# zhejz/TrafficBotsV1.5

Hardware: AMD Instinct MI355X
Metric: sim-agent-steps/sec (closed-loop rollout) (higher is better)
Workload: dtype f32 (split-bf16 MFMA products); 1 GPU; 64-agent/1024-polyline/128-light synthetic scene, 5-step teacher-forced prime + 1047-step closed-loop rollout; scenes_per_gpu=1, graph=True, steps_per_graph_replay=40, pre_roll_rollouts=32, one_queue_paired_launches=True, attn_mfma=False

## Files before the change

trafficbotsv1.5_amd/csrc/front.hip:

```cpp
#include <string.h>

#include "knn_core.h"
#include "tile_core.h"
#include "window_core.h"

using namespace tbx_tile;

namespace {

typedef Planes<16, 4> RPL;
constexpr int XLD = 132;
constexpr size_t WIN_BYTES = tbx_window::LDS_BYTES;
constexpr size_t POOL_OFF = WIN_BYTES;
constexpr size_t ROWP_OFF = POOL_OFF + 2 * D * sizeof(float);
constexpr size_t WIN_TOTAL = ROWP_OFF + 4 * 512;
constexpr size_t RIDER_TOTAL = 16 * XLD * sizeof(float) + 4 * RPL::PLANE;
constexpr size_t LDS_BYTES = WIN_TOTAL > RIDER_TOTAL ? WIN_TOTAL : RIDER_TOTAL;

struct FrontArgs {
  tbx_window_tile_t win;
  tbx_layer_tile_t lt;
  tbx_knn::KnnMulti knn;
  int n_win_blocks, n_rider_blocks, n_knn_blocks;
};

__device__ __forceinline__ void proj_rows(const tbx_layer_tile_t& t, const int block, const float* pooled, char* rowp) {
  const int tid = (int)threadIdx.x, lane = tid & 63;
  const int wave = __builtin_amdgcn_readfirstlane(tid >> 6);
  const int g4 = lane >> 4;
  const bool col0 = (lane & 15) == 0;
  const int c_out = 16 * wave + 4 * g4;
  constexpr int LO = 256;
  char* Ph = rowp;
  char* Pq = rowp + 1024;
  W wb[2];
  load_unit(wb[0], t.proj_image, wave, lane);
  load_unit(wb[1], t.proj_image, 8 + wave, lane);
  if (wave < 2) row1::ln_planes(pooled + wave * D, Ph + wave * 512, lane, t.proj_norm_eps, t.proj_norm_weight, t.proj_norm_bias);
  __syncthreads();
  const int64_t row0 = (int64_t)block * 2;
  const int nv = (t.n_rows - row0) < 2 ? (int)(t.n_rows - row0) : 2;
#pragma unroll
  for (int r = 0; r < 2; ++r) {
    const f32x4 q = row1::gemv4(wb[0], Ph + r * 512, LO, 0, g4) + wb[0].bias;
    if (col0) {
      row1::put4(Pq + r * 512, LO, c_out, q);
      if (r < nv) gst4(t.proj_out + (row0 + r) * (int64_t)t.ld_proj + c_out, q);
    }
  }
  load_unit(wb[0], t.proj_image, 16 + wave, lane);
#pragma unroll
  for (int kv = 0; kv < 2; ++kv) {
    const W& w = wb[1 - kv];
#pragma unroll
    for (int r = 0; r < 2; ++r) {
      const f32x4 y = row1::gemv4(w, Ph + r * 512, LO, 0, g4) + w.bias;
      if (col0 && r < nv) {
        gst4(t.proj_out + (row0 + r) * (int64_t)t.ld_proj + (1 + kv) * D + c_out, y);
        if (t.kv16_out != nullptr) {
          const bf16x4 h16 = __builtin_convertvector(y, bf16x4);
          *(TBX_GLOBAL u32x2*)((uint16_t*)t.kv16_out + (row0 + r) * (2 * D) + kv * D + c_out) = __builtin_bit_cast(u32x2, h16);
        }
      }
    }
    if (kv == 0) load_unit(wb[1], t.qfold_image, wave, lane);
  }
  __syncthreads();
  {
    const W& w = wb[1];
    const int h = wave >> 1;
#pragma unroll
    for (int st = 0; st < 4; ++st)
#pragma unroll
      for (int r = 0; r < 2; ++r) {
        Acc acc;
        acc.zero();
        row1::step(acc, w.hi[st], w.lo[st], Pq + r * 512, LO, h, g4);
        if (col0 && r < nv) gst4(t.proj_out + (row0 + r) * (int64_t)t.ld_proj + 3 * D + h * D + ((wave & 1) * 4 + st) * 16 + 4 * g4, acc.sum());
      }
  }
}

template <int DM, bool ADD>
__device__ __forceinline__ void front_body(const FrontArgs& a, int b, char* lds_c) {
  if (b < a.n_win_blocks) {
    float* pooled = (float*)(lds_c + POOL_OFF);
    tbx_window::window_body<DM, ADD>(a.win, b, lds_c, pooled);
    __syncthreads();
    proj_rows(a.lt, b, pooled, lds_c + ROWP_OFF);
    return;
  }
  b -= a.n_win_blocks;
  if (b < a.n_rider_blocks) {
    float* X = (float*)lds_c;
    char* Pa = (char*)(X + 16 * XLD);
    rider_tile<RPL, XLD>(a.lt, b, X, Pa, Pa + 2 * RPL::PLANE);
    return;
  }
  b -= a.n_rider_blocks;
  if (threadIdx.x < 256) tbx_knn::knn_multi_body(a.knn, b);
}

template <int DM, bool ADD>
__global__ __launch_bounds__(NT) void front_kernel(const FrontArgs a) {
  extern __shared__ __attribute__((aligned(16))) char lds_c[];
  front_body<DM, ADD>(a, (int)blockIdx.x, lds_c);
}

struct FrontPair {
  FrontArgs a, b;
  int n_b;
};
__global__ __launch_bounds__(NT) void front_pair_kernel(const FrontPair p) {
  extern __shared__ __attribute__((aligned(16))) char lds_c[];
  if ((int)blockIdx.x < p.n_b) front_body<128, true>(p.b, (int)blockIdx.x, lds_c);
  else front_body<64, false>(p.a, (int)blockIdx.x - p.n_b, lds_c);
}

static int front_fill(const tbx_front_t* args, FrontArgs& a, int& blocks) {
  if (args == nullptr) return TBX_ERR_ARG;
  const tbx_window_tile_t& w = args->win;
  const tbx_layer_tile_t& t = args->layer;
  if (w.n_groups <= 0 || w.attr == nullptr || w.pe == nullptr || w.row_invalid == nullptr || w.out == nullptr) return TBX_ERR_ARG;
  for (int i = 0; i < 3; ++i)
    if (w.in_images[i] == nullptr || w.pn_images[i] == nullptr) return TBX_ERR_ARG;
  if (w.window <= 0 || w.window > 16 || w.ld_attr % 4 != 0 || w.attr_cols <= 0 || w.attr_cols > 32 || w.attr_cols % 4 != 0 || w.attr_cols > w.ld_attr)
    return TBX_ERR_UNSUPPORTED;
  if (!((w.d_mlp == 64 && w.add_mode == 0) || (w.d_mlp == 128 && w.add_mode == 1))) return TBX_ERR_UNSUPPORTED;
  if (w.drop_thresh != 0u) return TBX_ERR_UNSUPPORTED;
  if ((((uintptr_t)w.attr) | ((uintptr_t)w.pe) | ((uintptr_t)w.out)) & 15) return TBX_ERR_ALIGN;
  if (t.x != w.out || t.n_rows != w.n_groups || t.attn_out != nullptr || t.linear1_image != nullptr || t.proj_n != 3 * D) return TBX_ERR_ARG;
  if (t.proj_image == nullptr || t.qfold_image == nullptr || t.proj_norm_weight == nullptr || t.proj_norm_bias == nullptr || t.proj_out == nullptr ||
      t.ld_proj < 7 * D || t.ld_proj % 4 != 0 || t.drop_thresh != 0u)
    return TBX_ERR_ARG;
  if (((uintptr_t)t.proj_out) & 15) return TBX_ERR_ALIGN;
  if (t.rider_rows < 0) return TBX_ERR_ARG;
  if (t.rider_rows > 0) {
    if ((t.rider_in == nullptr && t.rider_pose3 == nullptr) || t.rider_add == nullptr || t.rider_valid == nullptr || t.rider_out == nullptr)
      return TBX_ERR_ARG;
    if (t.rider_pose3 != nullptr && (t.rider_freqs_xy == nullptr || t.rider_freqs_yaw == nullptr)) return TBX_ERR_ARG;
    for (int i = 0; i < 4; ++i)
      if (t.rider_images[i] == nullptr) return TBX_ERR_ARG;
    if ((((uintptr_t)t.rider_in) | ((uintptr_t)t.rider_add) | ((uintptr_t)t.rider_out)) & 15) return TBX_ERR_ALIGN;
  }
  a.win = w, a.lt = t;
  a.n_win_blocks = (int)((w.n_groups + tbx_window::RT - 1) / tbx_window::RT);
  a.n_rider_blocks = (int)((t.rider_rows + 15) / 16);
  a.n_knn_blocks = 0;
  memset(&a.knn, 0, sizeof(a.knn));
  if (args->n_jobs > 0) {
    const int rc = tbx_knn::knn_multi_fill(args->jobs, args->n_jobs, args->freqs_xy, args->freqs_yaw, args->pe_dim, args->pe, a.knn, a.n_knn_blocks);
    if (rc != TBX_OK) return rc;
    for (int j = 0; j < args->n_jobs; ++j)
      if (args->jobs[j].emb != nullptr) return TBX_ERR_UNSUPPORTED;
  } else if (args->pe != nullptr) {
    return TBX_ERR_ARG;
  }
  blocks = a.n_win_blocks + a.n_rider_blocks + a.n_knn_blocks;
  return TBX_OK;
}

static bool front_lds_attr() {
  static tbx::PerDeviceOnce lds_attr;
  return lds_attr([&] { return !(hipFuncSetAttribute((const void*)front_kernel<64, false>, hipFuncAttributeMaxDynamicSharedMemorySize, (int)LDS_BYTES) != hipSuccess ||
        hipFuncSetAttribute((const void*)front_kernel<128, true>, hipFuncAttributeMaxDynamicSharedMemorySize, (int)LDS_BYTES) != hipSuccess ||
        hipFuncSetAttribute((const void*)front_pair_kernel, hipFuncAttributeMaxDynamicSharedMemorySize, (int)LDS_BYTES) != hipSuccess); });
}

}

extern "C" int tbx_front(const tbx_front_t* args, void* stream) {
  FrontArgs a;
  int blocks = 0;
  const int rc = front_fill(args, a, blocks);
  if (rc != TBX_OK) return rc;
  if (!front_lds_attr()) return TBX_ERR_LAUNCH;
  const dim3 grid((unsigned)blocks);
  if (args->win.d_mlp == 64)
    hipLaunchKernelGGL((front_kernel<64, false>), grid, dim3(NT), LDS_BYTES, (hipStream_t)stream, a);
  else
    hipLaunchKernelGGL((front_kernel<128, true>), grid, dim3(NT), LDS_BYTES, (hipStream_t)stream, a);
  return hipGetLastError() == hipSuccess ? TBX_OK : TBX_ERR_LAUNCH;
}

extern "C" int tbx_front_pair(const tbx_front_t* agents, const tbx_front_t* lights, void* stream) {
  FrontPair p;
  int na = 0, nb = 0;
  int rc = front_fill(agents, p.a, na);
  if (rc != TBX_OK) return rc;
  rc = front_fill(lights, p.b, nb);
  if (rc != TBX_OK) return rc;
  if (agents->win.d_mlp != 64 || lights->win.d_mlp != 128) return TBX_ERR_UNSUPPORTED;
  if (!front_lds_attr()) return TBX_ERR_LAUNCH;
  p.n_b = nb;
  hipLaunchKernelGGL(front_pair_kernel, dim3((unsigned)(na + nb)), dim3(NT), LDS_BYTES, (hipStream_t)stream, p);
  return hipGetLastError() == hipSuccess ? TBX_OK : TBX_ERR_LAUNCH;
}
```

trafficbotsv1.5_amd/csrc/knn_core.h:

```cpp
#pragma once
#include <hip/hip_runtime.h>
#include <limits.h>
#include <stdint.h>

#include "../../include/tbx_hip.h"
#include "tbx_common.h"

namespace tbx_knn {

struct KnnArgs {
  const float* src_pose;
  const uint8_t* src_invalid;
  const float* tgt_pose;
  const uint8_t* tgt_invalid;
  int32_t* idx;
  uint8_t* invalid;
  float* rel_pose;
  float* emb;
  const float* fxy;
  const float* fyaw;
  int n_rows, n_src, n_tgt, tgt_batch_div, k, pe_dim;
  float dist_limit;
};

__device__ __forceinline__ void rel_xy(float x1, float y1, float c, float s, float x2, float y2, float& rx, float& ry) {
  const float dx = __fsub_rn(x2, x1), dy = __fsub_rn(y2, y1);
  rx = __fadd_rn(__fmul_rn(dx, c), __fmul_rn(dy, s));
  ry = __fadd_rn(__fmul_rn(dx, -s), __fmul_rn(dy, c));
}

template <int MAXC, int WPR>
__device__ __forceinline__ void knn_rows(const KnnArgs& a, int block) {
  constexpr int RPB = 4 / WPR;
  __shared__ float rel_s[RPB][64][3];
  const int lane = threadIdx.x & 63;
  const int wv = threadIdx.x >> 6;
  const int wave = wv / WPR;
  const int wir = wv % WPR;
  const int row = block * RPB + wave;
  if (row >= a.n_rows) return;
  const int b = row / a.n_src;
  const int bt = b / a.tgt_batch_div;
  const float x1 = a.src_pose[row * 3 + 0], y1 = a.src_pose[row * 3 + 1], yaw1 = a.src_pose[row * 3 + 2];
  const bool inv1 = a.src_invalid[row] != 0;
  const float c = cosf(yaw1), s = sinf(yaw1);
  const float* tp = a.tgt_pose + (int64_t)bt * a.n_tgt * 3;
  const uint8_t* ti = a.tgt_invalid + (int64_t)bt * a.n_tgt;

  if (wir == 0) {
    uint32_t key[MAXC];
    float crx[MAXC], cry[MAXC], cyaw[MAXC];
    uint32_t tinv = 0;
    {
      float tx[MAXC], ty[MAXC];
      uint8_t tb[MAXC];
#pragma unroll
      for (int q = 0; q < MAXC; ++q) {
        const int j = min(lane + 64 * q, a.n_tgt - 1);
        tx[q] = tp[j * 3 + 0];
        ty[q] = tp[j * 3 + 1];
        cyaw[q] = tp[j * 3 + 2];
        tb[q] = ti[j];
      }
#pragma unroll
      for (int q = 0; q < MAXC; ++q) {
        const bool tin = tb[q] != 0;
        rel_xy(x1, y1, c, s, tx[q], ty[q], crx[q], cry[q]);
        cyaw[q] = __fsub_rn(cyaw[q], yaw1);
        tinv |= tin ? (1u << q) : 0u;
        const float dist = __fsqrt_rn(__fmaf_rn(cry[q], cry[q], __fmul_rn(crx[q], crx[q])));
        key[q] = (lane + 64 * q < a.n_tgt) ? __float_as_uint((inv1 || tin) ? INFINITY : dist) : 0xffffffffu;
      }
    }
    uint32_t kth = 0;
    for (int bit = 30; bit >= 0; --bit) {
      const uint32_t cand = kth | (1u << bit);
      int cnt = 0;
#pragma unroll
      for (int q = 0; q < MAXC; ++q) cnt += __popcll(__ballot(key[q] < cand));
      if (cnt < a.k) kth = cand;
    }
    int n_less = 0;
#pragma unroll
    for (int q = 0; q < MAXC; ++q) n_less += __popcll(__ballot(key[q] < kth));
    const int n_ties = a.k - n_less;
    const uint64_t lt_mask = (1ull << lane) - 1ull;
    int ties_before = 0, chosen_before = 0;
#pragma unroll
    for (int q = 0; q < MAXC; ++q) {
      const bool tie = key[q] == kth;
      const uint64_t tie_m = __ballot(tie);
      const bool take = key[q] < kth || (tie && ties_before + __popcll(tie_m & lt_mask) < n_ties);
      const uint64_t take_m = __ballot(take);
      if (take) {
        const int pos = chosen_before + __popcll(take_m & lt_mask);
        const int j = lane + 64 * q;
        const int64_t o = (int64_t)row * a.k + pos;
        const float dist = __uint_as_float(key[q]);
        a.idx[o] = j;
        a.invalid[o] = (((tinv >> q) & 1u) != 0 || dist > a.dist_limit) ? 1 : 0;
        const float rx = crx[q], ry = cry[q], ryaw = cyaw[q];
        rel_s[wave][pos][0] = rx;
        rel_s[wave][pos][1] = ry;
        rel_s[wave][pos][2] = ryaw;
        if (a.rel_pose != nullptr) {
          a.rel_pose[o * 3 + 0] = rx;
          a.rel_pose[o * 3 + 1] = ry;
          a.rel_pose[o * 3 + 2] = ryaw;
        }
      }
      ties_before += __popcll(tie_m);
      chosen_before += __popcll(take_m);
    }
  }
  if (a.emb == nullptr) return;
  if constexpr (WPR > 1)
    __syncthreads();
  else
    __builtin_amdgcn_wave_barrier();
  for (int t = wir; t < a.k; t += WPR) {
    const float x = rel_s[wave][t][0], y = rel_s[wave][t][1], yaw = rel_s[wave][t][2];
    tbx::pose_emb_write(a.emb + ((int64_t)row * a.k + t) * a.pe_dim, a.pe_dim, x, y, yaw, a.fxy, a.fyaw, lane, 64);
  }
}

constexpr int KNN_MAX_JOBS = 4;
struct PoseEmbedArgs {
  const float* pose3;
  const float *fxy, *fyaw;
  float* out;
  int64_t n;
  int pe_dim, ld, col_off;
};
struct KnnMulti {
  KnnArgs job[KNN_MAX_JOBS];
  int first_block[KNN_MAX_JOBS + 1];
  int n_jobs;
  PoseEmbedArgs pe;
};
__device__ __forceinline__ void knn_multi_body(const KnnMulti& m, const int bid) {
  if (bid >= m.first_block[KNN_MAX_JOBS]) {
    const int half = m.pe.pe_dim >> 1;
    const int64_t e = (int64_t)(bid - m.first_block[KNN_MAX_JOBS]) * 256 + threadIdx.x;
    if (e >= m.pe.n * half) return;
    const int64_t i = e / half;
    const int c = (int)(e - i * half);
    tbx::pose_emb_write(m.pe.out + i * m.pe.ld + m.pe.col_off, m.pe.pe_dim, m.pe.pose3[i * 3], m.pe.pose3[i * 3 + 1], m.pe.pose3[i * 3 + 2],
                        m.pe.fxy, m.pe.fyaw, c, half);
    return;
  }
  int j = 0;
  while (j + 1 < m.n_jobs && bid >= m.first_block[j + 1]) ++j;
  const KnnArgs& a = m.job[j];
  const int block = bid - m.first_block[j];
  if (a.n_tgt <= 128)
    knn_rows<2, 4>(a, block);
  else if (a.n_tgt <= 1024)
    knn_rows<16, 4>(a, block);
  else
    knn_rows<32, 4>(a, block);
}


inline int knn_multi_fill(const tbx_knn_job_t* jobs, int n_jobs, const float* freqs_xy, const float* freqs_yaw, int pe_dim,
                          const tbx_pose_embed_job_t* pe, KnnMulti& m, int& blocks) {
  if (!jobs || n_jobs <= 0 || n_jobs > KNN_MAX_JOBS) return TBX_ERR_ARG;
  m.n_jobs = n_jobs;
  m.pe = PoseEmbedArgs{nullptr, nullptr, nullptr, nullptr, 0, 0, 0, 0};
  if (pe != nullptr) {
    if (!pe->pose3 || !pe->freqs_xy || !pe->freqs_yaw || !pe->out || pe->n <= 0) return TBX_ERR_ARG;
    if ((pe->pe_dim != 64 && pe->pe_dim != 128) || pe->ld_out < pe->col_off + pe->pe_dim) return TBX_ERR_UNSUPPORTED;
    m.pe = PoseEmbedArgs{pe->pose3, pe->freqs_xy, pe->freqs_yaw, pe->out, pe->n, pe->pe_dim, pe->ld_out, pe->col_off};
  }
  blocks = 0;
  for (int j = 0; j < n_jobs; ++j) {
    const tbx_knn_job_t& q = jobs[j];
    if (!q.src_pose || !q.src_invalid || !q.tgt_pose || !q.tgt_invalid || !q.idx || !q.invalid) return TBX_ERR_ARG;
    if (q.n_batch <= 0 || q.n_src <= 0 || q.n_tgt <= 0 || q.tgt_batch_div <= 0 || q.n_batch % q.tgt_batch_div != 0) return TBX_ERR_ARG;
    if (q.k <= 0 || q.k >= q.n_tgt || q.k > 64 || q.n_tgt > 2048) return TBX_ERR_UNSUPPORTED;
    if (q.emb != nullptr && (!freqs_xy || !freqs_yaw || (pe_dim != 64 && pe_dim != 128))) return TBX_ERR_UNSUPPORTED;
    m.job[j] = KnnArgs{q.src_pose, q.src_invalid, q.tgt_pose, q.tgt_invalid, q.idx, q.invalid, q.rel_pose, q.emb, freqs_xy, freqs_yaw,
                       q.n_batch * q.n_src, q.n_src, q.n_tgt, q.tgt_batch_div, q.k, pe_dim, q.dist_limit};
    m.first_block[j] = blocks;
    blocks += q.n_batch * q.n_src;
  }
  for (int j = n_jobs; j <= KNN_MAX_JOBS; ++j) m.first_block[j] = blocks;
  for (int j = n_jobs; j < KNN_MAX_JOBS; ++j) m.job[j] = m.job[0];
  if (m.pe.n > 0) blocks += (int)((m.pe.n * (m.pe.pe_dim >> 1) + 255) / 256);
  return TBX_OK;
}

}
```

trafficbotsv1.5_amd/csrc/tile_core.h:

```cpp
#pragma once
#include <hip/hip_runtime.h>
#include <stdint.h>

#include "../../include/tbx_hip.h"
#include "drop_key.h"
#include "tbx_common.h"

#ifndef TBX_TILE_SINGLE
#define TBX_TILE_SINGLE 0
#endif
#if TBX_TILE_SINGLE
#define TBX_TILE_ENTRY(name) name##_bf16
#else
#define TBX_TILE_ENTRY(name) name
#endif

namespace tbx_tile {

typedef __bf16 bf16x8 __attribute__((ext_vector_type(8)));
typedef __bf16 bf16x4 __attribute__((ext_vector_type(4)));
typedef __bf16 bf16x2 __attribute__((ext_vector_type(2)));
typedef float f32x4 __attribute__((ext_vector_type(4)));
typedef float f32x2 __attribute__((ext_vector_type(2)));
typedef uint32_t u32x2 __attribute__((ext_vector_type(2)));

#define TBX_GLOBAL __attribute__((address_space(1)))

constexpr int NWAVE = 8, NT = NWAVE * 64, D = 128;
constexpr int UNIT = TBX_MFMA32_UNIT_FLOATS;

template <int R, int STEPS>
struct Planes {
  static constexpr int PRS = 16 * (STEPS | 1);
  static constexpr int PREG = ((R * PRS + 255) / 256) * 256;
  static constexpr int PLANE = 4 * PREG;
  static __device__ __forceinline__ int off(int row, int k) { return ((k >> 3) & 3) * PREG + row * PRS + (k >> 5) * 16 + (k & 7) * 2; }
  static __device__ __forceinline__ int lane_off(int lane, int r0) { return (lane >> 4) * PREG + (r0 + (lane & 15)) * PRS; }
};

struct Entry {
  const float* img;
  int32_t unit0, pad;
};

struct W {
  bf16x8 hi[4], lo[4];
  f32x4 bias;
};

__device__ __forceinline__ const TBX_GLOBAL float* unit_ptr(const float* img, int unit) {
  return (const TBX_GLOBAL float*)img + (int64_t)unit * UNIT;
}
__device__ __forceinline__ void load_unit(W& w, const float* img, int unit, int lane) {
  const TBX_GLOBAL float* base = unit_ptr(img, unit);
#ifdef TBX_ABL_NOLOAD
  base = unit_ptr(img, 0);
#endif
#pragma unroll
  for (int s = 0; s < 4; ++s) {
    w.hi[s] = *(const TBX_GLOBAL bf16x8*)(base + s * 512 + lane * 4);
#if !TBX_TILE_SINGLE
    w.lo[s] = *(const TBX_GLOBAL bf16x8*)(base + s * 512 + 256 + lane * 4);
#endif
  }
  w.bias = *(const TBX_GLOBAL f32x4*)(base + 2048 + (lane >> 4) * 4);
}
__device__ __forceinline__ void load_unit(W& w, const Entry& e, int wave, int lane) { load_unit(w, e.img, e.unit0 + wave, lane); }
__device__ __forceinline__ f32x4 unit_bias(const float* img, int unit, int s, int lane) {
  return *(const TBX_GLOBAL f32x4*)(unit_ptr(img, unit) + 2048 + s * 16 + (lane >> 4) * 4);
}

struct Acc {
  f32x4 hh, hl, lh;
  __device__ __forceinline__ void zero() { hh = hl = lh = (f32x4){0.f, 0.f, 0.f, 0.f}; }
  __device__ __forceinline__ f32x4 sum() const { return hh + (hl + lh); }
};

template <int PLANE>
__device__ __forceinline__ void mfma_step(Acc& a, const bf16x8 whi, const bf16x8 wlo, const char* act_hi, int step) {
  const bf16x8 xh = *(const bf16x8*)(act_hi + step * 16);
#if TBX_TILE_SINGLE
  a.hh = __builtin_amdgcn_mfma_f32_16x16x32_bf16(whi, xh, a.hh, 0, 0, 0);
  return;
#endif
  const bf16x8 xl = *(const bf16x8*)(act_hi + PLANE + step * 16);
#ifdef TBX_ABL_NOMFMA
  a.hh = __builtin_amdgcn_mfma_f32_16x16x32_bf16(whi, xh, a.hh, 0, 0, 0);
  a.hl[0] += (float)xl[0];
  a.lh[0] += (float)wlo[0];
#else
  a.hh = __builtin_amdgcn_mfma_f32_16x16x32_bf16(whi, xh, a.hh, 0, 0, 0);
  a.hl = __builtin_amdgcn_mfma_f32_16x16x32_bf16(whi, xl, a.hl, 0, 0, 0);
  a.lh = __builtin_amdgcn_mfma_f32_16x16x32_bf16(wlo, xh, a.lh, 0, 0, 0);
#endif
}

__device__ __forceinline__ void split4(const f32x4 v, u32x2& hi, u32x2& lo) {
  const bf16x4 h = __builtin_convertvector(v, bf16x4);
  const f32x4 r = v - __builtin_convertvector(h, f32x4);
  const bf16x4 l = __builtin_convertvector(r, bf16x4);
  hi = __builtin_bit_cast(u32x2, h);
  lo = __builtin_bit_cast(u32x2, l);
}

template <class PL>
__device__ __forceinline__ void planes_write4(char* p, int row, int c, const f32x4 v) {
  const int o = PL::off(row, c);
#if TBX_TILE_SINGLE
  *(u32x2*)(p + o) = __builtin_bit_cast(u32x2, __builtin_convertvector(v, bf16x4));
#else
  u32x2 hi, lo;
  split4(v, hi, lo);
  *(u32x2*)(p + o) = hi;
  *(u32x2*)(p + PL::PLANE + o) = lo;
#endif
}

__device__ __forceinline__ f32x4 drop4(f32x4 v, uint32_t base, const tbx_drop::StreamKey sk, uint32_t thresh, float scale) {
#pragma unroll
  for (int r = 0; r < 4; ++r) v[r] = tbx_drop::drop_mix(base + (uint32_t)r, sk.lo, sk.hi) >= thresh ? v[r] * scale : 0.f;
  return v;
}
struct DropKey4 {
  tbx_drop::StreamKey sk;
  uint32_t thresh;
  float scale;
  __device__ __forceinline__ void init(const uint64_t* seed, uint32_t site, uint32_t step, uint32_t thresh_, float scale_) {
    sk = tbx_drop::stream_key(*(const TBX_GLOBAL uint64_t*)seed, site, step);
    thresh = thresh_, scale = scale_;
  }
  __device__ __forceinline__ f32x4 apply(f32x4 v, int64_t row, int c, int n) const {
    return drop4(v, (uint32_t)row * (uint32_t)n + (uint32_t)c, sk, thresh, scale);
  }
};

__device__ __forceinline__ f32x4 gld4(const float* p) { return *(const TBX_GLOBAL f32x4*)p; }
__device__ __forceinline__ void gst4(float* p, const f32x4 v) { *(TBX_GLOBAL f32x4*)p = v; }
__device__ __forceinline__ f32x4 relu4(f32x4 v) {
  v[0] = fmaxf(v[0], 0.f), v[1] = fmaxf(v[1], 0.f), v[2] = fmaxf(v[2], 0.f), v[3] = fmaxf(v[3], 0.f);
  return v;
}


namespace row1 {
__device__ __forceinline__ void put4(char* P, int lo, int c, const f32x4 v) {
#if TBX_TILE_SINGLE
  *(u32x2*)(P + c * 2) = __builtin_bit_cast(u32x2, __builtin_convertvector(v, bf16x4));
#else
  u32x2 hi, l;
  split4(v, hi, l);
  *(u32x2*)(P + c * 2) = hi;
  *(u32x2*)(P + lo + c * 2) = l;
#endif
}
__device__ __forceinline__ void step(Acc& acc, const bf16x8 whi, const bf16x8 wlo, const char* P, int lo, int st, int g4) {
  const bf16x8 xh = *(const bf16x8*)(P + (st * 32 + g4 * 8) * 2);
  acc.hh = __builtin_amdgcn_mfma_f32_16x16x32_bf16(whi, xh, acc.hh, 0, 0, 0);
#if !TBX_TILE_SINGLE
  const bf16x8 xl = *(const bf16x8*)(P + lo + (st * 32 + g4 * 8) * 2);
  acc.hl = __builtin_amdgcn_mfma_f32_16x16x32_bf16(whi, xl, acc.hl, 0, 0, 0);
  acc.lh = __builtin_amdgcn_mfma_f32_16x16x32_bf16(wlo, xh, acc.lh, 0, 0, 0);
#endif
}
__device__ __forceinline__ f32x4 gemv4(const W& w, const char* P, int lo, int st0, int g4) {
  Acc acc;
  acc.zero();
#pragma unroll
  for (int st = 0; st < 4; ++st) step(acc, w.hi[st], w.lo[st], P, lo, st0 + st, g4);
  return acc.sum();
}
__device__ __forceinline__ void ln_planes(const float* src, char* P, int lane, float eps, const float* gamma, const float* beta) {
  float v[2], gm[2], bt[2];
#pragma unroll
  for (int q = 0; q < 2; ++q) {
    v[q] = src[lane + 64 * q];
    gm[q] = *(const TBX_GLOBAL float*)(gamma + lane + 64 * q);
    bt[q] = *(const TBX_GLOBAL float*)(beta + lane + 64 * q);
  }
  const float mean = tbx::wave_sum(v[0] + v[1]) / 128.f;
  const float d0 = v[0] - mean, d1 = v[1] - mean;
  const float var = tbx::wave_sum(d0 * d0 + d1 * d1) / 128.f;
  const float rstd = 1.0f / sqrtf(var + eps);
#pragma unroll
  for (int q = 0; q < 2; ++q) {
    const float y = (v[q] - mean) * rstd * gm[q] + bt[q];
    const __bf16 h = (__bf16)y;
    *(__bf16*)(P + 2 * (lane + 64 * q)) = h;
#if !TBX_TILE_SINGLE
    *(__bf16*)(P + 256 + 2 * (lane + 64 * q)) = (__bf16)(y - (float)h);
#endif
  }
}
}

template <class PL, int XLD>
__device__ __forceinline__ void rider_tile(const tbx_layer_tile_t& t, int tile, float* X, char* Pa, char* Pb) {
  constexpr int ROWS = 16;
  constexpr int PLANE = PL::PLANE;
  const int tid = (int)threadIdx.x, lane = tid & 63;
  const int wave = __builtin_amdgcn_readfirstlane(tid >> 6);
  const int j = lane & 15, g = lane >> 4;
  const int64_t row0 = (int64_t)tile * ROWS;
  const int nv = (t.rider_rows - row0) < ROWS ? (int)(t.rider_rows - row0) : ROWS;
  const bool row_ok = j < nv;
  const int64_t grow = row0 + (row_ok ? j : 0);
  const int aoff = PL::lane_off(lane, 0);
  const int c_out = 16 * wave + 4 * g;
  W wb[2];
  load_unit(wb[0], t.rider_images[0], wave, lane);
  load_unit(wb[1], t.rider_images[1], wave, lane);
  const f32x4 add = gld4(t.rider_add + grow * D + c_out);
  const bool ok = *(const TBX_GLOBAL uint8_t*)(t.rider_valid + grow) != 0;
  {
    const int r = tid >> 5, c4 = tid & 31;
    f32x4 v = {0.f, 0.f, 0.f, 0.f};
    if (t.rider_pose3 != nullptr) {
      if (r < nv) {
        const TBX_GLOBAL float* p3 = (const TBX_GLOBAL float*)t.rider_pose3 + (row0 + r) * 3;
        tbx::pose_emb_write(X + r * XLD, D, p3[0], p3[1], p3[2], t.rider_freqs_xy, t.rider_freqs_yaw, c4, 32);
      }
      __syncthreads();
      if (r < nv) v = *(const f32x4*)(X + r * XLD + c4 * 4);
    } else if (r < nv) {
      v = gld4(t.rider_in + (row0 + r) * D + c4 * 4);
    }
    planes_write4<PL>(Pa, r, c4 * 4, v);
  }
  __syncthreads();
  {
    Acc acc;
    acc.zero();
#pragma unroll
    for (int s = 0; s < 4; ++s) mfma_step<PLANE>(acc, wb[0].hi[s], wb[0].lo[s], Pa + aoff, s);
    planes_write4<PL>(Pb, j, c_out, add + (acc.sum() + wb[0].bias));
    load_unit(wb[0], t.rider_images[2], wave, lane);
  }
  __syncthreads();
  {
    Acc acc;
    acc.zero();
#pragma unroll
    for (int s = 0; s < 4; ++s) mfma_step<PLANE>(acc, wb[1].hi[s], wb[1].lo[s], Pb + aoff, s);
    planes_write4<PL>(Pa, j, c_out, relu4(acc.sum() + wb[1].bias));
    load_unit(wb[1], t.rider_images[3], wave, lane);
  }
  __syncthreads();
  {
    Acc acc;
    acc.zero();
#pragma unroll
    for (int s = 0; s < 4; ++s) mfma_step<PLANE>(acc, wb[0].hi[s], wb[0].lo[s], Pa + aoff, s);
    planes_write4<PL>(Pb, j, c_out, relu4(acc.sum() + wb[0].bias));
  }
  __syncthreads();
  {
    Acc acc;
    acc.zero();
#pragma unroll
    for (int s = 0; s < 4; ++s) mfma_step<PLANE>(acc, wb[1].hi[s], wb[1].lo[s], Pb + aoff, s);
    f32x4 v = relu4(acc.sum() + wb[1].bias);
    if (!ok) v = (f32x4){0.f, 0.f, 0.f, 0.f};
    if (row_ok) gst4(t.rider_out + grow * D + c_out, v);
  }
}


}
```

trafficbotsv1.5_amd/csrc/tile_window.hip:

```cpp
#include "window_core.h"

using namespace tbx_tile;

namespace {

using namespace tbx_window;

struct WindowArgs {
  tbx_window_tile_t t;
};

template <int DM, bool ADD>
__global__ __launch_bounds__(NT) void tile_window_kernel(const WindowArgs a) {
  extern __shared__ __attribute__((aligned(16))) char lds_c[];
  window_body<DM, ADD>(a.t, (int)blockIdx.x, lds_c, nullptr);
}

}

extern "C" int TBX_TILE_ENTRY(tbx_window_tile)(const tbx_window_tile_t* args, void* stream) {
  if (args == nullptr || args->n_groups <= 0) return TBX_ERR_ARG;
  const tbx_window_tile_t& t = *args;
  if (t.attr == nullptr || t.pe == nullptr || t.row_invalid == nullptr || t.out == nullptr) return TBX_ERR_ARG;
  for (int i = 0; i < 3; ++i)
    if (t.in_images[i] == nullptr || t.pn_images[i] == nullptr) return TBX_ERR_ARG;
  if (t.window <= 0 || t.window > 16 || t.ld_attr % 4 != 0 || t.attr_cols <= 0 || t.attr_cols > 32 || t.attr_cols % 4 != 0 ||
      t.attr_cols > t.ld_attr)
    return TBX_ERR_UNSUPPORTED;
  if (!((t.d_mlp == 64 && t.add_mode == 0) || (t.d_mlp == 128 && t.add_mode == 1))) return TBX_ERR_UNSUPPORTED;
  if ((((uintptr_t)t.attr) | ((uintptr_t)t.pe) | ((uintptr_t)t.out)) & 15) return TBX_ERR_ALIGN;
  if (t.drop_thresh != 0u && t.drop_seed == nullptr) return TBX_ERR_ARG;
  WindowArgs a;
  a.t = t;
  static tbx::PerDeviceOnce lds_attr;
  if (!lds_attr([&] { return !(hipFuncSetAttribute((const void*)tile_window_kernel<64, false>, hipFuncAttributeMaxDynamicSharedMemorySize, (int)LDS_BYTES) != hipSuccess ||
        hipFuncSetAttribute((const void*)tile_window_kernel<128, true>, hipFuncAttributeMaxDynamicSharedMemorySize, (int)LDS_BYTES) != hipSuccess); })) return TBX_ERR_LAUNCH;
  const dim3 grid((unsigned)((t.n_groups + RT - 1) / RT));
  if (t.d_mlp == 64)
    hipLaunchKernelGGL((tile_window_kernel<64, false>), grid, dim3(NT), LDS_BYTES, (hipStream_t)stream, a);
  else
    hipLaunchKernelGGL((tile_window_kernel<128, true>), grid, dim3(NT), LDS_BYTES, (hipStream_t)stream, a);
  return hipGetLastError() == hipSuccess ? TBX_OK : TBX_ERR_LAUNCH;
}
```

trafficbotsv1.5_amd/csrc/window_core.h:

```cpp
#pragma once
#include "tile_core.h"

namespace tbx_window {
using namespace tbx_tile;


constexpr int RT = 2;
constexpr int ROWS = 16 * RT;
typedef Planes<ROWS, 4> PL;
constexpr int PLANE = PL::PLANE;
constexpr size_t LDS_BYTES = 4 * PLANE;

__device__ __forceinline__ float row16_max(float v) {
  v = fmaxf(v, tbx::dpp<tbx::DPP_XOR1>(v));
  v = fmaxf(v, tbx::dpp<tbx::DPP_XOR2>(v));
  v = fmaxf(v, tbx::dpp<tbx::DPP_HALF_MIRROR>(v));
  return fmaxf(v, tbx::dpp<tbx::DPP_MIRROR>(v));
}

template <int DM, bool ADD>
__device__ __forceinline__ void window_body(const tbx_window_tile_t& t, const int block, char* lds_c, float* pooled) {
  char* P0 = lds_c;
  char* P1 = P0 + 2 * PLANE;
  const int tid = (int)threadIdx.x, lane = tid & 63;
  const int wave = __builtin_amdgcn_readfirstlane(tid >> 6);
  const int j = lane & 15, g = lane >> 4;
  const int nt = wave & 3, rt = wave >> 2;
  const int64_t grp0 = (int64_t)block * RT;
  const int Wn = t.window;
  const int aoff = PL::lane_off(lane, rt * 16);
  const int c_out = 16 * nt + 4 * g;
  const int64_t grp = grp0 + rt;
  const bool grp_ok = grp < t.n_groups;
  bool inv = true;
  if (grp_ok && j < Wn) inv = *(const TBX_GLOBAL uint8_t*)(t.row_invalid + grp * Wn + j) != 0;

  W wb[2];
  if (tid < ROWS * 8) {
    const int r = tid >> 3, c4 = tid & 7;
    const int64_t gq = grp0 + (r >> 4);
    f32x4 v = {0.f, 0.f, 0.f, 0.f};
    if (gq < t.n_groups && (r & 15) < Wn && c4 * 4 < t.attr_cols) v = gld4(t.attr + (gq * Wn + (r & 15)) * (int64_t)t.ld_attr + c4 * 4);
    planes_write4<PL>(P0, r, c4 * 4, v);
  }
  if constexpr (!ADD) {
    const int r = tid >> 4, c4 = tid & 15;
    const int64_t gq = grp0 + (r >> 4);
    f32x4 v = {0.f, 0.f, 0.f, 0.f};
    if (gq < t.n_groups && (r & 15) < Wn) v = gld4(t.pe + (gq * Wn + (r & 15)) * (int64_t)64 + c4 * 4);
    planes_write4<PL>(P1, r, 64 + c4 * 4, v);
  }
  if constexpr (DM == 64) {
    load_unit(wb[0], t.in_images[0], 0, lane);
    const f32x4 b_in0 = unit_bias(t.in_images[0], 0, nt, lane);
    __syncthreads();
    {
      load_unit(wb[1], t.in_images[1], nt >> 1, lane);
      Acc acc;
      acc.zero();
      const W& w = wb[0];
      const bf16x8 wh = nt == 0 ? w.hi[0] : (nt == 1 ? w.hi[1] : (nt == 2 ? w.hi[2] : w.hi[3]));
      const bf16x8 wl = nt == 0 ? w.lo[0] : (nt == 1 ? w.lo[1] : (nt == 2 ? w.lo[2] : w.lo[3]));
      mfma_step<PLANE>(acc, wh, wl, P0 + aoff, 0);
      planes_write4<PL>(P1, rt * 16 + j, c_out, relu4(acc.sum() + b_in0));
    }
    __syncthreads();
#define TBX_IN64(CUR, SRC, DST, RELU, NEXT_IMG, NEXT_UNIT, BIAS_IMG)                                      \
  do {                                                                                                    \
    const f32x4 bias = unit_bias(BIAS_IMG, nt >> 1, 2 * (nt & 1), lane);                                  \
    load_unit(wb[1 - (CUR)], NEXT_IMG, NEXT_UNIT, lane);                                                  \
    Acc acc;                                                                                              \
    acc.zero();                                                                                           \
    const W& w = wb[CUR];                                                                                 \
    const bool odd = (nt & 1) != 0;                                                                       \
    mfma_step<PLANE>(acc, odd ? w.hi[2] : w.hi[0], odd ? w.lo[2] : w.lo[0], (SRC) + aoff, 0);             \
    mfma_step<PLANE>(acc, odd ? w.hi[3] : w.hi[1], odd ? w.lo[3] : w.lo[1], (SRC) + aoff, 1);             \
    f32x4 v = acc.sum() + bias;                                                                           \
    if (RELU) v = relu4(v);                                                                               \
    planes_write4<PL>(DST, rt * 16 + j, c_out, v);                                                        \
  } while (0)
    TBX_IN64(1, P1, P0, true, t.in_images[2], nt >> 1, t.in_images[1]);
    __syncthreads();
    TBX_IN64(0, P0, P1, false, t.pn_images[0], nt, t.in_images[2]);
#undef TBX_IN64
    __syncthreads();
  } else {
    const int c8 = 16 * wave + 4 * g;
    load_unit(wb[0], t.in_images[0], wave >> 2, lane);
    const f32x4 b_in0 = unit_bias(t.in_images[0], wave >> 2, wave & 3, lane);
    __syncthreads();
    {
      load_unit(wb[1], t.in_images[1], wave, lane);
      const W& w = wb[0];
      const int q = wave & 3;
      const bf16x8 wh = q == 0 ? w.hi[0] : (q == 1 ? w.hi[1] : (q == 2 ? w.hi[2] : w.hi[3]));
      const bf16x8 wl = q == 0 ? w.lo[0] : (q == 1 ? w.lo[1] : (q == 2 ? w.lo[2] : w.lo[3]));
#pragma unroll
      for (int r2 = 0; r2 < RT; ++r2) {
        Acc acc;
        acc.zero();
        mfma_step<PLANE>(acc, wh, wl, P0 + PL::lane_off(lane, r2 * 16), 0);
        planes_write4<PL>(P1, r2 * 16 + j, c8, relu4(acc.sum() + b_in0));
      }
    }
    __syncthreads();
    {
      load_unit(wb[0], t.in_images[2], wave, lane);
      const W& w = wb[1];
#pragma unroll
      for (int r2 = 0; r2 < RT; ++r2) {
        Acc acc;
        acc.zero();
#pragma unroll
        for (int s2 = 0; s2 < 4; ++s2) mfma_step<PLANE>(acc, w.hi[s2], w.lo[s2], P1 + PL::lane_off(lane, r2 * 16), s2);
        planes_write4<PL>(P0, r2 * 16 + j, c8, relu4(acc.sum() + w.bias));
      }
    }
    __syncthreads();
    {
      load_unit(wb[1], t.pn_images[0], nt, lane);
      const W& w = wb[0];
#pragma unroll
      for (int r2 = 0; r2 < RT; ++r2) {
        Acc acc;
        acc.zero();
#pragma unroll
        for (int s2 = 0; s2 < 4; ++s2) mfma_step<PLANE>(acc, w.hi[s2], w.lo[s2], P0 + PL::lane_off(lane, r2 * 16), s2);
        f32x4 v = acc.sum() + w.bias;
        const int64_t gq = grp0 + r2;
        if (gq < t.n_groups) v += gld4(t.pe + gq * (int64_t)D + c8);
        planes_write4<PL>(P1, r2 * 16 + j, c8, v);
      }
    }
    __syncthreads();
  }
#define TBX_PN(CUR, SRC, DST, LAST, NEXT_IMG, LAYER)                                                      \
  do {                                                                                                    \
    if (!(LAST)) load_unit(wb[1 - (CUR)], NEXT_IMG, nt, lane);                                            \
    Acc acc;                                                                                              \
    acc.zero();                                                                                           \
    const W& w = wb[CUR];                                                                                 \
    _Pragma("unroll") for (int s = 0; s < 4; ++s) mfma_step<PLANE>(acc, w.hi[s], w.lo[s], (SRC) + aoff, s); \
    f32x4 h = relu4(acc.sum() + w.bias);                                                                  \
    if (t.drop_thresh != 0u && j < Wn) {                                                                  \
      DropKey4 dk;                                                                                        \
      dk.init(t.drop_seed, (uint32_t)t.drop_site[LAYER], (uint32_t)t.drop_step, t.drop_thresh, t.drop_scale); \
      h = dk.apply(h, grp * Wn + j, c_out, 64);                                                           \
    }                                                                                                     \
    f32x4 m;                                                                                              \
    _Pragma("unroll") for (int r = 0; r < 4; ++r) m[r] = row16_max(inv ? -INFINITY : h[r]);               \
    _Pragma("unroll") for (int r = 0; r < 4; ++r) m[r] = m[r] == -INFINITY ? 0.f : m[r];                  \
    if (!(LAST)) {                                                                                        \
      const f32x4 z = {0.f, 0.f, 0.f, 0.f};                                                               \
      planes_write4<PL>(DST, rt * 16 + j, c_out, inv ? z : h);                                            \
      planes_write4<PL>(DST, rt * 16 + j, 64 + c_out, inv ? z : m);                                       \
    } else if (j == 0) {                                                                                  \
      if (grp_ok) {                                                                                       \
        gst4(t.out + grp * D + c_out, m);                                                                 \
        gst4(t.out + grp * D + 64 + c_out, m);                                                            \
      }                                                                                                   \
      if (pooled != nullptr) {                                                                            \
        *(f32x4*)(pooled + rt * D + c_out) = m;                                                           \
        *(f32x4*)(pooled + rt * D + 64 + c_out) = m;                                                      \
      }                                                                                                   \
    }                                                                                                     \
  } while (0)
  TBX_PN(1, P1, P0, false, t.pn_images[1], 0);
  __syncthreads();
  TBX_PN(0, P0, P1, false, t.pn_images[2], 1);
  __syncthreads();
  TBX_PN(1, P1, P0, true, t.pn_images[2], 2);
#undef TBX_PN
}


}
```

Measured before the change: 538,800 sim-agent-steps/s.

## Slim front-kernel arguments, hoist loads, and specialize knn/dropout paths

Replaces the large per-half argument structs with compact Win/Proj/Rider argument packs and a 64-byte scalar head, so the kernel loads less kernel-argument data. Global loads for attributes, positional encodings, biases and LayerNorm parameters are issued earlier, with clamped unconditional addressing, so their latency overlaps weight loading. Dropout becomes a compile-time template flag, and knn jobs are dispatched per job with a BIG template parameter and the embedding work skipped. Optional clock64 stage instrumentation is added behind TBX_STAGE_CLOCK. In exchange, register pressure rises from the hoisted loads and the number of kernel instantiations grows.

```diff
diff --git a/trafficbotsv1.5_amd/csrc/front.hip b/trafficbotsv1.5_amd/csrc/front.hip
--- a/trafficbotsv1.5_amd/csrc/front.hip
+++ b/trafficbotsv1.5_amd/csrc/front.hip
@@ -1,4 +1,16 @@
 #include <string.h>
+
+#ifdef TBX_STAGE_CLOCK
+#include <hip/hip_runtime.h>
+__device__ unsigned long long g_front_clk[4 * 32];
+__device__ int g_front_clk_blk[4];
+__shared__ int g_front_clk_slot;
+#define TBX_FRONT_CLK(i)                                                                 \
+  do {                                                                                   \
+    if (threadIdx.x == 0 && g_front_clk_slot >= 0) g_front_clk[g_front_clk_slot * 32 + (i)] = clock64(); \
+  } while (0)
+#define TBX_FRONT_CLK_LOADS() asm volatile("s_waitcnt vmcnt(0)" ::: "memory")
+#endif
 
 #include "knn_core.h"
 #include "tile_core.h"
@@ -17,14 +29,47 @@
 constexpr size_t RIDER_TOTAL = 16 * XLD * sizeof(float) + 4 * RPL::PLANE;
 constexpr size_t LDS_BYTES = WIN_TOTAL > RIDER_TOTAL ? WIN_TOTAL : RIDER_TOTAL;
 
-struct FrontArgs {
-  tbx_window_tile_t win;
-  tbx_layer_tile_t lt;
-  tbx_knn::KnnMulti knn;
-  int n_win_blocks, n_rider_blocks, n_knn_blocks;
-};
-
-__device__ __forceinline__ void proj_rows(const tbx_layer_tile_t& t, const int block, const float* pooled, char* rowp) {
+struct WinArgs {
+  const float *attr, *pe;
+  const uint8_t* row_invalid;
+  float* out;
+  const float* in_images[3];
+  const float* pn_images[3];
+  int64_t n_groups;
+  int32_t window, ld_attr, attr_cols, pad_;
+};
+struct ProjArgs {
+  const float *proj_norm_weight, *proj_norm_bias, *proj_image, *qfold_image;
+  float* proj_out;
+  void* kv16_out;
+  int64_t n_rows;
+  int32_t ld_proj;
+  float proj_norm_eps;
+};
+struct RiderArgs {
+  const float *rider_in, *rider_add, *rider_pose3, *rider_freqs_xy, *rider_freqs_yaw;
+  const uint8_t* rider_valid;
+  float* rider_out;
+  const float* rider_images[4];
+  int64_t rider_rows;
+};
+struct HalfArgs {
+  WinArgs win;
+  ProjArgs proj;
+  RiderArgs rider;
+  tbx_knn::KnnArgs job[tbx_knn::KNN_MAX_JOBS];
+  tbx_knn::PoseEmbedArgs pe;
+};
+struct FrontHead {
+  int32_t n0;
+  int32_t n_win[2], n_rider[2];
+  int32_t fb[2][tbx_knn::KNN_MAX_JOBS];
+  int32_t pad_[3];
+};
+static_assert(sizeof(FrontHead) == 64, "the head is one 64-byte scalar load");
+
+__device__ __forceinline__ void proj_rows(const ProjArgs& t, const int block, const float* pooled, char* rowp, const float (&lg)[2],
+                                          const float (&lb)[2]) {
   const int tid = (int)threadIdx.x, lane = tid & 63;
   const int wave = __builtin_amdgcn_readfirstlane(tid >> 6);
   const int g4 = lane >> 4;
@@ -36,10 +81,12 @@
   W wb[2];
   load_unit(wb[0], t.proj_image, wave, lane);
   load_unit(wb[1], t.proj_image, 8 + wave, lane);
-  if (wave < 2) row1::ln_planes(pooled + wave * D, Ph + wave * 512, lane, t.proj_norm_eps, t.proj_norm_weight, t.proj_norm_bias);
+  if (wave < 2) row1::ln_planes(pooled + wave * D, Ph + wave * 512, lane, t.proj_norm_eps, lg, lb);
   __syncthreads();
+  TBX_FRONT_CLK(8);
   const int64_t row0 = (int64_t)block * 2;
   const int nv = (t.n_rows - row0) < 2 ? (int)(t.n_rows - row0) : 2;
+  const bool kv16 = t.kv16_out != nullptr;
 #pragma unroll
   for (int r = 0; r < 2; ++r) {
     const f32x4 q = row1::gemv4(wb[0], Ph + r * 512, LO, 0, g4) + wb[0].bias;
@@ -48,6 +95,7 @@
       if (r < nv) gst4(t.proj_out + (row0 + r) * (int64_t)t.ld_proj + c_out, q);
     }
   }
+  TBX_FRONT_CLK(9);
   load_unit(wb[0], t.proj_image, 16 + wave, lane);
 #pragma unroll
   for (int kv = 0; kv < 2; ++kv) {
@@ -57,7 +105,7 @@
       const f32x4 y = row1::gemv4(w, Ph + r * 512, LO, 0, g4) + w.bias;
       if (col0 && r < nv) {
         gst4(t.proj_out + (row0 + r) * (int64_t)t.ld_proj + (1 + kv) * D + c_out, y);
-        if (t.kv16_out != nullptr) {
+        if (kv16) {
           const bf16x4 h16 = __builtin_convertvector(y, bf16x4);
           *(TBX_GLOBAL u32x2*)((uint16_t*)t.kv16_out + (row0 + r) * (2 * D) + kv * D + c_out) = __builtin_bit_cast(u32x2, h16);
         }
@@ -66,6 +114,7 @@
     if (kv == 0) load_unit(wb[1], t.qfold_image, wave, lane);
   }
   __syncthreads();
+  TBX_FRONT_CLK(10);
   {
     const W& w = wb[1];
     const int h = wave >> 1;
@@ -79,45 +128,74 @@
         if (col0 && r < nv) gst4(t.proj_out + (row0 + r) * (int64_t)t.ld_proj + 3 * D + h * D + ((wave & 1) * 4 + st) * 16 + 4 * g4, acc.sum());
       }
   }
-}
-
-template <int DM, bool ADD>
-__device__ __forceinline__ void front_body(const FrontArgs& a, int b, char* lds_c) {
-  if (b < a.n_win_blocks) {
+  TBX_FRONT_CLK(11);
+}
+
+template <int DM, bool ADD, bool BIG>
+__device__ __forceinline__ void front_half(const HalfArgs& a, int b, const int n_win, const int n_rider, const int f1, const int f2, const int f3,
+                                           const int f4, char* lds_c) {
+  if (b < n_win) {
+    float lg[2], lb[2];
+    row1::ln_params(a.proj.proj_norm_weight, a.proj.proj_norm_bias, (int)threadIdx.x & 63, lg, lb);
     float* pooled = (float*)(lds_c + POOL_OFF);
-    tbx_window::window_body<DM, ADD>(a.win, b, lds_c, pooled);
+    tbx_window::window_body<DM, ADD, false>(a.win, b, lds_c, pooled);
     __syncthreads();
-    proj_rows(a.lt, b, pooled, lds_c + ROWP_OFF);
+    TBX_FRONT_CLK(7);
+    proj_rows(a.proj, b, pooled, lds_c + ROWP_OFF, lg, lb);
     return;
   }
-  b -= a.n_win_blocks;
-  if (b < a.n_rider_blocks) {
+  b -= n_win;
+  if (b < n_rider) {
     float* X = (float*)lds_c;
     char* Pa = (char*)(X + 16 * XLD);
-    rider_tile<RPL, XLD>(a.lt, b, X, Pa, Pa + 2 * RPL::PLANE);
+    rider_tile<RPL, XLD>(a.rider, b, X, Pa, Pa + 2 * RPL::PLANE);
     return;
   }
-  b -= a.n_rider_blocks;
-  if (threadIdx.x < 256) tbx_knn::knn_multi_body(a.knn, b);
-}
-
-template <int DM, bool ADD>
-__global__ __launch_bounds__(NT) void front_kernel(const FrontArgs a) {
+  b -= n_rider;
+  if (threadIdx.x >= 256) return;
+  if (b >= f4) tbx_knn::pose_embed_block(a.pe, b - f4);
+  else if (b < f1) tbx_knn::knn_job_block<BIG, false>(a.job[0], b);
+  else if (b < f2) tbx_knn::knn_job_block<BIG, false>(a.job[1], b - f1);
+  else if (b < f3) tbx_knn::knn_job_block<BIG, false>(a.job[2], b - f2);
+  else tbx_knn::knn_job_block<BIG, false>(a.job[3], b - f3);
+}
+
+struct FrontArgs {
+  FrontHead h;
+  HalfArgs a;
+};
+template <int DM, bool ADD, bool BIG>
+__global__ __launch_bounds__(NT) void front_kernel(const FrontArgs p) {
   extern __shared__ __attribute__((aligned(16))) char lds_c[];
-  front_body<DM, ADD>(a, (int)blockIdx.x, lds_c);
+#ifdef TBX_STAGE_CLOCK
+  if (threadIdx.x == 0) g_front_clk_slot = -1;
+#endif
+  const FrontHead h = p.h;
+  front_half<DM, ADD, BIG>(p.a, (int)blockIdx.x, h.n_win[0], h.n_rider[0], h.fb[0][0], h.fb[0][1], h.fb[0][2], h.fb[0][3], lds_c);
 }
 
 struct FrontPair {
-  FrontArgs a, b;
-  int n_b;
-};
+  FrontHead h;
+  HalfArgs m[2];
+};
+template <bool BIG>
 __global__ __launch_bounds__(NT) void front_pair_kernel(const FrontPair p) {
   extern __shared__ __attribute__((aligned(16))) char lds_c[];
-  if ((int)blockIdx.x < p.n_b) front_body<128, true>(p.b, (int)blockIdx.x, lds_c);
-  else front_body<64, false>(p.a, (int)blockIdx.x - p.n_b, lds_c);
-}
-
-static int front_fill(const tbx_front_t* args, FrontArgs& a, int& blocks) {
+#ifdef TBX_STAGE_CLOCK
+  if (threadIdx.x == 0) {
+    int slot = -1;
+    for (int q = 0; q < 4; ++q)
+      if (g_front_clk_blk[q] == (int)blockIdx.x) slot = q;
+    g_front_clk_slot = slot;
+  }
+#endif
+  const FrontHead h = p.h;
+  const int b = (int)blockIdx.x;
+  if (b < h.n0) front_half<128, true, BIG>(p.m[0], b, h.n_win[0], h.n_rider[0], h.fb[0][0], h.fb[0][1], h.fb[0][2], h.fb[0][3], lds_c);
+  else front_half<64, false, BIG>(p.m[1], b - h.n0, h.n_win[1], h.n_rider[1], h.fb[1][0], h.fb[1][1], h.fb[1][2], h.fb[1][3], lds_c);
+}
+
+static int front_fill(const tbx_front_t* args, FrontHead& h, const int half, HalfArgs& a, int& blocks, bool& big) {
   if (args == nullptr) return TBX_ERR_ARG;
   const tbx_window_tile_t& w = args->win;
   const tbx_layer_tile_t& t = args->layer;
@@ -143,56 +221,102 @@
       if (t.rider_images[i] == nullptr) return TBX_ERR_ARG;
     if ((((uintptr_t)t.rider_in) | ((uintptr_t)t.rider_add) | ((uintptr_t)t.rider_out)) & 15) return TBX_ERR_ALIGN;
   }
-  a.win = w, a.lt = t;
-  a.n_win_blocks = (int)((w.n_groups + tbx_window::RT - 1) / tbx_window::RT);
-  a.n_rider_blocks = (int)((t.rider_rows + 15) / 16);
-  a.n_knn_blocks = 0;
-  memset(&a.knn, 0, sizeof(a.knn));
+  a.win = WinArgs{w.attr, w.pe, w.row_invalid, w.out, {w.in_images[0], w.in_images[1], w.in_images[2]}, {w.pn_images[0], w.pn_images[1], w.pn_images[2]},
+                  w.n_groups, w.window, w.ld_attr, w.attr_cols, 0};
+  a.proj = ProjArgs{t.proj_norm_weight, t.proj_norm_bias, t.proj_image, t.qfold_image, t.proj_out, t.kv16_out, t.n_rows, t.ld_proj, t.proj_norm_eps};
+  a.rider = RiderArgs{t.rider_in, t.rider_add, t.rider_pose3, t.rider_freqs_xy, t.rider_freqs_yaw, t.rider_valid, t.rider_out,
+                      {t.rider_images[0], t.rider_images[1], t.rider_images[2], t.rider_images[3]}, t.rider_rows};
+  h.n_win[half] = (int)((w.n_groups + tbx_window::RT - 1) / tbx_window::RT);
+  h.n_rider[half] = (int)((t.rider_rows + 15) / 16);
+  int n_knn_blocks = 0;
+  tbx_knn::KnnMulti m;
+  memset(&m, 0, sizeof(m));
   if (args->n_jobs > 0) {
-    const int rc = tbx_knn::knn_multi_fill(args->jobs, args->n_jobs, args->freqs_xy, args->freqs_yaw, args->pe_dim, args->pe, a.knn, a.n_knn_blocks);
+    const int rc = tbx_knn::knn_multi_fill(args->jobs, args->n_jobs, args->freqs_xy, args->freqs_yaw, args->pe_dim, args->pe, m, n_knn_blocks);
     if (rc != TBX_OK) return rc;
-    for (int j = 0; j < args->n_jobs; ++j)
+    for (int j = 0; j < args->n_jobs; ++j) {
       if (args->jobs[j].emb != nullptr) return TBX_ERR_UNSUPPORTED;
+      big = big || args->jobs[j].n_tgt > 1024;
+    }
   } else if (args->pe != nullptr) {
     return TBX_ERR_ARG;
   }
-  blocks = a.n_win_blocks + a.n_rider_blocks + a.n_knn_blocks;
+  for (int j = 0; j < tbx_knn::KNN_MAX_JOBS; ++j) a.job[j] = m.job[j], h.fb[half][j] = m.first_block[j + 1];
+  a.pe = m.pe;
+  blocks = h.n_win[half] + h.n_rider[half] + n_knn_blocks;
   return TBX_OK;
 }
 
 static bool front_lds_attr() {
   static tbx::PerDeviceOnce lds_attr;
-  return lds_attr([&] { return !(hipFuncSetAttribute((const void*)front_kernel<64, false>, hipFuncAttributeMaxDynamicSharedMemorySize, (int)LDS_BYTES) != hipSuccess ||
-        hipFuncSetAttribute((const void*)front_kernel<128, true>, hipFuncAttributeMaxDynamicSharedMemorySize, (int)LDS_BYTES) != hipSuccess ||
-        hipFuncSetAttribute((const void*)front_pair_kernel, hipFuncAttributeMaxDynamicSharedMemorySize, (int)LDS_BYTES) != hipSuccess); });
-}
-
-}
+  return lds_attr([&] {
+    const void* ks[] = {(const void*)front_kernel<64, false, false>, (const void*)front_kernel<64, false, true>, (const void*)front_kernel<128, true, false>,
+                        (const void*)front_kernel<128, true, true>, (const void*)front_pair_kernel<false>, (const void*)front_pair_kernel<true>};
+    for (const void* k : ks)
+      if (hipFuncSetAttribute(k, hipFuncAttributeMaxDynamicSharedMemorySize, (int)LDS_BYTES) != hipSuccess) return false;
+    return true;
+  });
+}
+
+}
+
+#define TBX_FRONT_LAUNCH(K, GRID, ARGS)                                                                             \
+  do {                                                                                                              \
+    if (big) hipLaunchKernelGGL((K<true>), GRID, dim3(NT), LDS_BYTES, (hipStream_t)stream, ARGS);                   \
+    else hipLaunchKernelGGL((K<false>), GRID, dim3(NT), LDS_BYTES, (hipStream_t)stream, ARGS);                      \
+  } while (0)
+template <bool BIG>
+static constexpr auto front_cat_kernel = front_kernel<64, false, BIG>;
+template <bool BIG>
+static constexpr auto front_add_kernel = front_kernel<128, true, BIG>;
 
 extern "C" int tbx_front(const tbx_front_t* args, void* stream) {
-  FrontArgs a;
+  FrontArgs p;
+  memset(&p.h, 0, sizeof(p.h));
   int blocks = 0;
-  const int rc = front_fill(args, a, blocks);
+  bool big = false;
+  const int rc = front_fill(args, p.h, 0, p.a, blocks, big);
   if (rc != TBX_OK) return rc;
   if (!front_lds_attr()) return TBX_ERR_LAUNCH;
+  p.h.n0 = blocks;
   const dim3 grid((unsigned)blocks);
-  if (args->win.d_mlp == 64)
-    hipLaunchKernelGGL((front_kernel<64, false>), grid, dim3(NT), LDS_BYTES, (hipStream_t)stream, a);
-  else
-    hipLaunchKernelGGL((front_kernel<128, true>), grid, dim3(NT), LDS_BYTES, (hipStream_t)stream, a);
+  if (args->win.d_mlp == 64) TBX_FRONT_LAUNCH(front_cat_kernel, grid, p);
+  else TBX_FRONT_LAUNCH(front_add_kernel, grid, p);
   return hipGetLastError() == hipSuccess ? TBX_OK : TBX_ERR_LAUNCH;
 }
 
 extern "C" int tbx_front_pair(const tbx_front_t* agents, const tbx_front_t* lights, void* stream) {
   FrontPair p;
+  memset(&p.h, 0, sizeof(p.h));
   int na = 0, nb = 0;
-  int rc = front_fill(agents, p.a, na);
+  bool big = false;
+  int rc = front_fill(agents, p.h, 1, p.m[1], na, big);
   if (rc != TBX_OK) return rc;
-  rc = front_fill(lights, p.b, nb);
+  rc = front_fill(lights, p.h, 0, p.m[0], nb, big);
   if (rc != TBX_OK) return rc;
   if (agents->win.d_mlp != 64 || lights->win.d_mlp != 128) return TBX_ERR_UNSUPPORTED;
   if (!front_lds_attr()) return TBX_ERR_LAUNCH;
-  p.n_b = nb;
-  hipLaunchKernelGGL(front_pair_kernel, dim3((unsigned)(na + nb)), dim3(NT), LDS_BYTES, (hipStream_t)stream, p);
+  p.h.n0 = nb;
+#ifdef TBX_STAGE_CLOCK
+  {
+    int sj = 0;
+    for (int j = 0; j < agents->n_jobs; ++j)
+      if (p.m[1].job[j].n_tgt == 1024) sj = j;
+    const int base = nb + p.h.n_win[1] + p.h.n_rider[1];
+    const int blk[4] = {0, nb, agents->n_jobs > 0 ? base + (sj > 0 ? p.h.fb[1][sj - 1] : 0) : -1, p.h.n_rider[1] > 0 ? nb + p.h.n_win[1] : -1};
+    if (hipMemcpyToSymbol(HIP_SYMBOL(g_front_clk_blk), blk, sizeof(blk)) != hipSuccess) return TBX_ERR_LAUNCH;
+  }
+#endif
+  TBX_FRONT_LAUNCH(front_pair_kernel, dim3((unsigned)(na + nb)), p);
   return hipGetLastError() == hipSuccess ? TBX_OK : TBX_ERR_LAUNCH;
 }
+#undef TBX_FRONT_LAUNCH
+
+#ifdef TBX_STAGE_CLOCK
+extern "C" int tbx_debug_front_dump(unsigned long long* host_out) {
+  static const unsigned long long z[4 * 32] = {};
+  if (hipDeviceSynchronize() != hipSuccess) return -1;
+  if (hipMemcpyFromSymbol(host_out, HIP_SYMBOL(g_front_clk), sizeof(z)) != hipSuccess) return -1;
+  return hipMemcpyToSymbol(HIP_SYMBOL(g_front_clk), z, sizeof(z)) == hipSuccess ? 0 : -1;
+}
+#endif
diff --git a/trafficbotsv1.5_amd/csrc/knn_core.h b/trafficbotsv1.5_amd/csrc/knn_core.h
--- a/trafficbotsv1.5_amd/csrc/knn_core.h
+++ b/trafficbotsv1.5_amd/csrc/knn_core.h
@@ -5,6 +5,11 @@
 
 #include "../../include/tbx_hip.h"
 #include "tbx_common.h"
+
+#ifndef TBX_FRONT_CLK
+#define TBX_FRONT_CLK(i)
+#define TBX_FRONT_CLK_LOADS()
+#endif
 
 namespace tbx_knn {
 
@@ -29,7 +34,7 @@
   ry = __fadd_rn(__fmul_rn(dx, -s), __fmul_rn(dy, c));
 }
 
-template <int MAXC, int WPR>
+template <int MAXC, int WPR, bool EMB = true>
 __device__ __forceinline__ void knn_rows(const KnnArgs& a, int block) {
   constexpr int RPB = 4 / WPR;
   __shared__ float rel_s[RPB][64][3];
@@ -39,15 +44,17 @@
   const int wir = wv % WPR;
   const int row = block * RPB + wave;
   if (row >= a.n_rows) return;
+  if constexpr (!EMB)
+    if (wir != 0) return;
   const int b = row / a.n_src;
   const int bt = b / a.tgt_batch_div;
   const float x1 = a.src_pose[row * 3 + 0], y1 = a.src_pose[row * 3 + 1], yaw1 = a.src_pose[row * 3 + 2];
-  const bool inv1 = a.src_invalid[row] != 0;
-  const float c = cosf(yaw1), s = sinf(yaw1);
+  const uint8_t inv1_b = a.src_invalid[row];
   const float* tp = a.tgt_pose + (int64_t)bt * a.n_tgt * 3;
   const uint8_t* ti = a.tgt_invalid + (int64_t)bt * a.n_tgt;
 
   if (wir == 0) {
+    TBX_FRONT_CLK(16);
     uint32_t key[MAXC];
     float crx[MAXC], cry[MAXC], cyaw[MAXC];
     uint32_t tinv = 0;
@@ -62,6 +69,10 @@
         cyaw[q] = tp[j * 3 + 2];
         tb[q] = ti[j];
       }
+      TBX_FRONT_CLK_LOADS();
+      TBX_FRONT_CLK(17);
+      const bool inv1 = inv1_b != 0;
+      const float c = cosf(yaw1), s = sinf(yaw1);
 #pragma unroll
       for (int q = 0; q < MAXC; ++q) {
         const bool tin = tb[q] != 0;
@@ -80,6 +91,7 @@
       for (int q = 0; q < MAXC; ++q) cnt += __popcll(__ballot(key[q] < cand));
       if (cnt < a.k) kth = cand;
     }
+    TBX_FRONT_CLK(18);
     int n_less = 0;
 #pragma unroll
     for (int q = 0; q < MAXC; ++q) n_less += __popcll(__ballot(key[q] < kth));
@@ -100,9 +112,11 @@
         a.idx[o] = j;
         a.invalid[o] = (((tinv >> q) & 1u) != 0 || dist > a.dist_limit) ? 1 : 0;
         const float rx = crx[q], ry = cry[q], ryaw = cyaw[q];
-        rel_s[wave][pos][0] = rx;
-        rel_s[wave][pos][1] = ry;
-        rel_s[wave][pos][2] = ryaw;
+        if constexpr (EMB) {
+          rel_s[wave][pos][0] = rx;
+          rel_s[wave][pos][1] = ry;
+          rel_s[wave][pos][2] = ryaw;
+        }
         if (a.rel_pose != nullptr) {
           a.rel_pose[o * 3 + 0] = rx;
           a.rel_pose[o * 3 + 1] = ry;
@@ -112,7 +126,9 @@
       ties_before += __popcll(tie_m);
       chosen_before += __popcll(take_m);
     }
-  }
+    TBX_FRONT_CLK(19);
+  }
+  if constexpr (!EMB) return;
   if (a.emb == nullptr) return;
   if constexpr (WPR > 1)
     __syncthreads();
@@ -138,27 +154,32 @@
   int n_jobs;
   PoseEmbedArgs pe;
 };
+__device__ __forceinline__ void pose_embed_block(const PoseEmbedArgs& pe, const int block) {
+  const int half = pe.pe_dim >> 1;
+  const int64_t e = (int64_t)block * 256 + threadIdx.x;
+  if (e >= pe.n * half) return;
+  const int64_t i = e / half;
+  const int c = (int)(e - i * half);
+  tbx::pose_emb_write(pe.out + i * pe.ld + pe.col_off, pe.pe_dim, pe.pose3[i * 3], pe.pose3[i * 3 + 1], pe.pose3[i * 3 + 2], pe.fxy, pe.fyaw, c, half);
+}
+template <bool BIG, bool EMB>
+__device__ __forceinline__ void knn_job_block(const KnnArgs& a, const int block) {
+  if (a.n_tgt <= 128) {
+    knn_rows<2, 4, EMB>(a, block);
+  } else if (!BIG || a.n_tgt <= 1024) {
+    knn_rows<16, 4, EMB>(a, block);
+  } else {
+    if constexpr (BIG) knn_rows<32, 4, EMB>(a, block);
+  }
+}
 __device__ __forceinline__ void knn_multi_body(const KnnMulti& m, const int bid) {
   if (bid >= m.first_block[KNN_MAX_JOBS]) {
-    const int half = m.pe.pe_dim >> 1;
-    const int64_t e = (int64_t)(bid - m.first_block[KNN_MAX_JOBS]) * 256 + threadIdx.x;
-    if (e >= m.pe.n * half) return;
-    const int64_t i = e / half;
-    const int c = (int)(e - i * half);
-    tbx::pose_emb_write(m.pe.out + i * m.pe.ld + m.pe.col_off, m.pe.pe_dim, m.pe.pose3[i * 3], m.pe.pose3[i * 3 + 1], m.pe.pose3[i * 3 + 2],
-                        m.pe.fxy, m.pe.fyaw, c, half);
+    pose_embed_block(m.pe, bid - m.first_block[KNN_MAX_JOBS]);
     return;
   }
   int j = 0;
   while (j + 1 < m.n_jobs && bid >= m.first_block[j + 1]) ++j;
-  const KnnArgs& a = m.job[j];
-  const int block = bid - m.first_block[j];
-  if (a.n_tgt <= 128)
-    knn_rows<2, 4>(a, block);
-  else if (a.n_tgt <= 1024)
-    knn_rows<16, 4>(a, block);
-  else
-    knn_rows<32, 4>(a, block);
+  knn_job_block<true, true>(m.job[j], bid - m.first_block[j]);
 }
 
 
diff --git a/trafficbotsv1.5_amd/csrc/tile_core.h b/trafficbotsv1.5_amd/csrc/tile_core.h
--- a/trafficbotsv1.5_amd/csrc/tile_core.h
+++ b/trafficbotsv1.5_amd/csrc/tile_core.h
@@ -25,6 +25,11 @@
 typedef uint32_t u32x2 __attribute__((ext_vector_type(2)));
 
 #define TBX_GLOBAL __attribute__((address_space(1)))
+
+#ifndef TBX_FRONT_CLK
+#define TBX_FRONT_CLK(i)
+#define TBX_FRONT_CLK_LOADS()
+#endif
 
 constexpr int NWAVE = 8, NT = NWAVE * 64, D = 128;
 constexpr int UNIT = TBX_MFMA32_UNIT_FLOATS;
@@ -169,14 +174,17 @@
   for (int st = 0; st < 4; ++st) step(acc, w.hi[st], w.lo[st], P, lo, st0 + st, g4);
   return acc.sum();
 }
-__device__ __forceinline__ void ln_planes(const float* src, char* P, int lane, float eps, const float* gamma, const float* beta) {
-  float v[2], gm[2], bt[2];
+__device__ __forceinline__ void ln_params(const float* gamma, const float* beta, int lane, float (&gm)[2], float (&bt)[2]) {
 #pragma unroll
   for (int q = 0; q < 2; ++q) {
-    v[q] = src[lane + 64 * q];
     gm[q] = *(const TBX_GLOBAL float*)(gamma + lane + 64 * q);
     bt[q] = *(const TBX_GLOBAL float*)(beta + lane + 64 * q);
   }
+}
+__device__ __forceinline__ void ln_planes(const float* src, char* P, int lane, float eps, const float (&gm)[2], const float (&bt)[2]) {
+  float v[2];
+#pragma unroll
+  for (int q = 0; q < 2; ++q) v[q] = src[lane + 64 * q];
   const float mean = tbx::wave_sum(v[0] + v[1]) / 128.f;
   const float d0 = v[0] - mean, d1 = v[1] - mean;
   const float var = tbx::wave_sum(d0 * d0 + d1 * d1) / 128.f;
@@ -193,8 +201,8 @@
 }
 }
 
-template <class PL, int XLD>
-__device__ __forceinline__ void rider_tile(const tbx_layer_tile_t& t, int tile, float* X, char* Pa, char* Pb) {
+template <class PL, int XLD, class T>
+__device__ __forceinline__ void rider_tile(const T& t, int tile, float* X, char* Pa, char* Pb) {
   constexpr int ROWS = 16;
   constexpr int PLANE = PL::PLANE;
   const int tid = (int)threadIdx.x, lane = tid & 63;
@@ -206,27 +214,34 @@
   const int64_t grow = row0 + (row_ok ? j : 0);
   const int aoff = PL::lane_off(lane, 0);
   const int c_out = 16 * wave + 4 * g;
+  TBX_FRONT_CLK(20);
+  const int r = tid >> 5, c4 = tid & 31;
+  const bool pose = t.rider_pose3 != nullptr;
+  const int64_t rin = row0 + (r < nv ? r : 0);
+  float p3[3] = {0.f, 0.f, 0.f};
+  f32x4 v = {0.f, 0.f, 0.f, 0.f};
+  if (pose) {
+#pragma unroll
+    for (int q = 0; q < 3; ++q) p3[q] = *((const TBX_GLOBAL float*)t.rider_pose3 + rin * 3 + q);
+  } else {
+    v = gld4(t.rider_in + rin * D + c4 * 4);
+  }
+  const f32x4 add = gld4(t.rider_add + grow * D + c_out);
+  const bool ok = *(const TBX_GLOBAL uint8_t*)(t.rider_valid + grow) != 0;
   W wb[2];
   load_unit(wb[0], t.rider_images[0], wave, lane);
   load_unit(wb[1], t.rider_images[1], wave, lane);
-  const f32x4 add = gld4(t.rider_add + grow * D + c_out);
-  const bool ok = *(const TBX_GLOBAL uint8_t*)(t.rider_valid + grow) != 0;
-  {
-    const int r = tid >> 5, c4 = tid & 31;
-    f32x4 v = {0.f, 0.f, 0.f, 0.f};
-    if (t.rider_pose3 != nullptr) {
-      if (r < nv) {
-        const TBX_GLOBAL float* p3 = (const TBX_GLOBAL float*)t.rider_pose3 + (row0 + r) * 3;
-        tbx::pose_emb_write(X + r * XLD, D, p3[0], p3[1], p3[2], t.rider_freqs_xy, t.rider_freqs_yaw, c4, 32);
-      }
+  {
+    if (pose) {
+      if (r < nv) tbx::pose_emb_write(X + r * XLD, D, p3[0], p3[1], p3[2], t.rider_freqs_xy, t.rider_freqs_yaw, c4, 32);
       __syncthreads();
       if (r < nv) v = *(const f32x4*)(X + r * XLD + c4 * 4);
-    } else if (r < nv) {
-      v = gld4(t.rider_in + (row0 + r) * D + c4 * 4);
     }
+    if (r >= nv) v = (f32x4){0.f, 0.f, 0.f, 0.f};
     planes_write4<PL>(Pa, r, c4 * 4, v);
   }
   __syncthreads();
+  TBX_FRONT_CLK(21);
   {
     Acc acc;
     acc.zero();
@@ -236,6 +251,7 @@
     load_unit(wb[0], t.rider_images[2], wave, lane);
   }
   __syncthreads();
+  TBX_FRONT_CLK(22);
   {
     Acc acc;
     acc.zero();
@@ -245,6 +261,7 @@
     load_unit(wb[1], t.rider_images[3], wave, lane);
   }
   __syncthreads();
+  TBX_FRONT_CLK(23);
   {
     Acc acc;
     acc.zero();
@@ -253,6 +270,7 @@
     planes_write4<PL>(Pb, j, c_out, relu4(acc.sum() + wb[0].bias));
   }
   __syncthreads();
+  TBX_FRONT_CLK(24);
   {
     Acc acc;
     acc.zero();
@@ -262,7 +280,8 @@
     if (!ok) v = (f32x4){0.f, 0.f, 0.f, 0.f};
     if (row_ok) gst4(t.rider_out + grow * D + c_out, v);
   }
-}
-
-
-}
+  TBX_FRONT_CLK(25);
+}
+
+
+}
diff --git a/trafficbotsv1.5_amd/csrc/tile_window.hip b/trafficbotsv1.5_amd/csrc/tile_window.hip
--- a/trafficbotsv1.5_amd/csrc/tile_window.hip
+++ b/trafficbotsv1.5_amd/csrc/tile_window.hip
@@ -13,7 +13,8 @@
 template <int DM, bool ADD>
 __global__ __launch_bounds__(NT) void tile_window_kernel(const WindowArgs a) {
   extern __shared__ __attribute__((aligned(16))) char lds_c[];
-  window_body<DM, ADD>(a.t, (int)blockIdx.x, lds_c, nullptr);
+  if (a.t.drop_thresh != 0u) window_body<DM, ADD, true>(a.t, (int)blockIdx.x, lds_c, nullptr);
+  else window_body<DM, ADD, false>(a.t, (int)blockIdx.x, lds_c, nullptr);
 }
 
 }
diff --git a/trafficbotsv1.5_amd/csrc/window_core.h b/trafficbotsv1.5_amd/csrc/window_core.h
--- a/trafficbotsv1.5_amd/csrc/window_core.h
+++ b/trafficbotsv1.5_amd/csrc/window_core.h
@@ -18,8 +18,8 @@
   return fmaxf(v, tbx::dpp<tbx::DPP_MIRROR>(v));
 }
 
-template <int DM, bool ADD>
-__device__ __forceinline__ void window_body(const tbx_window_tile_t& t, const int block, char* lds_c, float* pooled) {
+template <int DM, bool ADD, bool DROP, class T>
+__device__ __forceinline__ void window_body(const T& t, const int block, char* lds_c, float* pooled) {
   char* P0 = lds_c;
   char* P1 = P0 + 2 * PLANE;
   const int tid = (int)threadIdx.x, lane = tid & 63;
@@ -36,24 +36,39 @@
   if (grp_ok && j < Wn) inv = *(const TBX_GLOBAL uint8_t*)(t.row_invalid + grp * Wn + j) != 0;
 
   W wb[2];
-  if (tid < ROWS * 8) {
-    const int r = tid >> 3, c4 = tid & 7;
+  TBX_FRONT_CLK(0);
+  const f32x4 zero4 = {0.f, 0.f, 0.f, 0.f};
+  f32x4 v_attr, v_pe = zero4;
+  {
+    const int r = (tid >> 3) & (ROWS - 1), c4 = tid & 7;
     const int64_t gq = grp0 + (r >> 4);
-    f32x4 v = {0.f, 0.f, 0.f, 0.f};
-    if (gq < t.n_groups && (r & 15) < Wn && c4 * 4 < t.attr_cols) v = gld4(t.attr + (gq * Wn + (r & 15)) * (int64_t)t.ld_attr + c4 * 4);
-    planes_write4<PL>(P0, r, c4 * 4, v);
+    const bool ok = gq < t.n_groups && (r & 15) < Wn && c4 * 4 < t.attr_cols;
+    const int64_t gc = gq < t.n_groups ? gq : t.n_groups - 1;
+    const int rc = (r & 15) < Wn ? (r & 15) : Wn - 1, cc = c4 * 4 < t.attr_cols ? c4 * 4 : t.attr_cols - 4;
+    v_attr = gld4(t.attr + (gc * Wn + rc) * (int64_t)t.ld_attr + cc);
+    if (!ok) v_attr = zero4;
   }
   if constexpr (!ADD) {
     const int r = tid >> 4, c4 = tid & 15;
     const int64_t gq = grp0 + (r >> 4);
-    f32x4 v = {0.f, 0.f, 0.f, 0.f};
-    if (gq < t.n_groups && (r & 15) < Wn) v = gld4(t.pe + (gq * Wn + (r & 15)) * (int64_t)64 + c4 * 4);
-    planes_write4<PL>(P1, r, 64 + c4 * 4, v);
+    const bool ok = gq < t.n_groups && (r & 15) < Wn;
+    const int64_t gc = ok ? gq : t.n_groups - 1;
+    const int rc = ok ? (r & 15) : 0;
+    v_pe = gld4(t.pe + (gc * Wn + rc) * (int64_t)64 + c4 * 4);
+    if (!ok) v_pe = zero4;
   }
+  auto write_inputs = [&] {
+    if (tid < ROWS * 8) planes_write4<PL>(P0, tid >> 3, (tid & 7) * 4, v_attr);
+    if constexpr (!ADD) planes_write4<PL>(P1, tid >> 4, 64 + (tid & 15) * 4, v_pe);
+  };
   if constexpr (DM == 64) {
+    const f32x4 b_in0 = unit_bias(t.in_images[0], 0, nt, lane);
+    const f32x4 b_in1 = unit_bias(t.in_images[1], nt >> 1, 2 * (nt & 1), lane);
+    const f32x4 b_in2 = unit_bias(t.in_images[2], nt >> 1, 2 * (nt & 1), lane);
     load_unit(wb[0], t.in_images[0], 0, lane);
-    const f32x4 b_in0 = unit_bias(t.in_images[0], 0, nt, lane);
-    __syncthreads();
+    write_inputs();
+    __syncthreads();
+  TBX_FRONT_CLK(1);
     {
       load_unit(wb[1], t.in_images[1], nt >> 1, lane);
       Acc acc;
@@ -65,9 +80,10 @@
       planes_write4<PL>(P1, rt * 16 + j, c_out, relu4(acc.sum() + b_in0));
     }
     __syncthreads();
-#define TBX_IN64(CUR, SRC, DST, RELU, NEXT_IMG, NEXT_UNIT, BIAS_IMG)                                      \
+  TBX_FRONT_CLK(2);
+#define TBX_IN64(CUR, SRC, DST, RELU, NEXT_IMG, NEXT_UNIT, BIAS)                                          \
   do {                                                                                                    \
-    const f32x4 bias = unit_bias(BIAS_IMG, nt >> 1, 2 * (nt & 1), lane);                                  \
+    const f32x4 bias = BIAS;                                                                              \
     load_unit(wb[1 - (CUR)], NEXT_IMG, NEXT_UNIT, lane);                                                  \
     Acc acc;                                                                                              \
     acc.zero();                                                                                           \
@@ -79,16 +95,26 @@
     if (RELU) v = relu4(v);                                                                               \
     planes_write4<PL>(DST, rt * 16 + j, c_out, v);                                                        \
   } while (0)
-    TBX_IN64(1, P1, P0, true, t.in_images[2], nt >> 1, t.in_images[1]);
-    __syncthreads();
-    TBX_IN64(0, P0, P1, false, t.pn_images[0], nt, t.in_images[2]);
+    TBX_IN64(1, P1, P0, true, t.in_images[2], nt >> 1, b_in1);
+    __syncthreads();
+  TBX_FRONT_CLK(3);
+    TBX_IN64(0, P0, P1, false, t.pn_images[0], nt, b_in2);
 #undef TBX_IN64
     __syncthreads();
+  TBX_FRONT_CLK(4);
   } else {
     const int c8 = 16 * wave + 4 * g;
+    const f32x4 b_in0 = unit_bias(t.in_images[0], wave >> 2, wave & 3, lane);
+    f32x4 feat[RT];
+#pragma unroll
+    for (int r2 = 0; r2 < RT; ++r2) {
+      const int64_t gq = grp0 + r2 < t.n_groups ? grp0 + r2 : t.n_groups - 1;
+      feat[r2] = gld4(t.pe + gq * (int64_t)D + c8);
+    }
     load_unit(wb[0], t.in_images[0], wave >> 2, lane);
-    const f32x4 b_in0 = unit_bias(t.in_images[0], wave >> 2, wave & 3, lane);
-    __syncthreads();
+    write_inputs();
+    __syncthreads();
+  TBX_FRONT_CLK(1);
     {
       load_unit(wb[1], t.in_images[1], wave, lane);
       const W& w = wb[0];
@@ -104,6 +130,7 @@
       }
     }
     __syncthreads();
+  TBX_FRONT_CLK(2);
     {
       load_unit(wb[0], t.in_images[2], wave, lane);
       const W& w = wb[1];
@@ -117,6 +144,7 @@
       }
     }
     __syncthreads();
+  TBX_FRONT_CLK(3);
     {
       load_unit(wb[1], t.pn_images[0], nt, lane);
       const W& w = wb[0];
@@ -128,11 +156,12 @@
         for (int s2 = 0; s2 < 4; ++s2) mfma_step<PLANE>(acc, w.hi[s2], w.lo[s2], P0 + PL::lane_off(lane, r2 * 16), s2);
         f32x4 v = acc.sum() + w.bias;
         const int64_t gq = grp0 + r2;
-        if (gq < t.n_groups) v += gld4(t.pe + gq * (int64_t)D + c8);
+        if (gq < t.n_groups) v += feat[r2];
         planes_write4<PL>(P1, r2 * 16 + j, c8, v);
       }
     }
     __syncthreads();
+  TBX_FRONT_CLK(4);
   }
 #define TBX_PN(CUR, SRC, DST, LAST, NEXT_IMG, LAYER)                                                      \
   do {                                                                                                    \
@@ -142,7 +171,7 @@
     const W& w = wb[CUR];                                                                                 \
     _Pragma("unroll") for (int s = 0; s < 4; ++s) mfma_step<PLANE>(acc, w.hi[s], w.lo[s], (SRC) + aoff, s); \
     f32x4 h = relu4(acc.sum() + w.bias);                                                                  \
-    if (t.drop_thresh != 0u && j < Wn) {                                                                  \
+    if constexpr (DROP) if (j < Wn) {                                                                     \
       DropKey4 dk;                                                                                        \
       dk.init(t.drop_seed, (uint32_t)t.drop_site[LAYER], (uint32_t)t.drop_step, t.drop_thresh, t.drop_scale); \
       h = dk.apply(h, grp * Wn + j, c_out, 64);                                                           \
@@ -167,8 +196,10 @@
   } while (0)
   TBX_PN(1, P1, P0, false, t.pn_images[1], 0);
   __syncthreads();
+  TBX_FRONT_CLK(5);
   TBX_PN(0, P0, P1, false, t.pn_images[2], 1);
   __syncthreads();
+  TBX_FRONT_CLK(6);
   TBX_PN(1, P1, P0, true, t.pn_images[2], 2);
 #undef TBX_PN
 }
```

Measured after the change: 544,300 sim-agent-steps/s (median of 6 runs). 1.01x the previous value.
